# haoheliu/voicefixer_main

Measured on NVIDIA H100. Metric: clips_per_sec_10s_44k1, higher is better.
Workload: dtype f16 tensor-core (UNet: hi/lo split, fp32-grade; vocoder: hi-only), f32 accumulate

## Files before the change

voicefixer_main_b200/csrc/gemm_tc.cu:

```cuda
#include "gemm.cuh"
#include "ptx.cuh"

namespace vf {

namespace {

constexpr int kRowValid = 1, kRowPad = 2;

struct RowInfo {
  uint32_t orow;
  uint32_t flags;
};


__device__ __forceinline__ void epi_bar_sync(int nthreads) {
  asm volatile("bar.sync 1, %0;" ::"r"(nthreads) : "memory");
}
__device__ __forceinline__ void wg_bar_sync(int wg) {
  asm volatile("bar.sync %0, 128;" ::"r"(2 + wg) : "memory");
}

struct ChunkDesc {
  int a_c;
  int a_off;
  uint32_t kk;
  uint32_t flags;
};

struct TileCoord {
  int nt, mi, img;
  __device__ __forceinline__ TileCoord(uint32_t tile, const GemmTcParams& P, int n_tiles, int m_tiles) {
    const uint32_t mt = fast_div(tile, (uint32_t)n_tiles, P.magic_n);
    nt = (int)(tile - mt * (uint32_t)n_tiles);
    const uint32_t im = fast_div(mt, (uint32_t)m_tiles, P.magic_m);
    img = (int)im;
    mi = (int)(mt - im * (uint32_t)m_tiles);
  }
};

}

__device__ __forceinline__ void pack_hi(const float (&v)[32], uint32_t (&hi)[16]) {
#pragma unroll
  for (int i = 0; i < 16; ++i) {
    const __half2 h = __floats2half2_rn(v[2 * i], v[2 * i + 1]);
    hi[i] = *reinterpret_cast<const uint32_t*>(&h);
  }
}
__device__ __forceinline__ void pack_hi_lo(const float (&v)[32], uint32_t (&hi)[16], uint32_t (&lo)[16]) {
#pragma unroll
  for (int i = 0; i < 16; ++i) {
    const __half2 h = __floats2half2_rn(v[2 * i], v[2 * i + 1]);
    hi[i] = *reinterpret_cast<const uint32_t*>(&h);
    lo[i] = residual_h2(v[2 * i], v[2 * i + 1], hi[i]);
  }
}

template <bool TWO>
__device__ __forceinline__ void pack8(const float (&v)[32], const int i, uint4& h, uint4& l) {
  uint32_t hw[4], lw[4];
#pragma unroll
  for (int k = 0; k < 4; ++k) {
    const __half2 h2 = __floats2half2_rn(v[8 * i + 2 * k], v[8 * i + 2 * k + 1]);
    hw[k] = *reinterpret_cast<const uint32_t*>(&h2);
    if (TWO) lw[k] = residual_h2(v[8 * i + 2 * k], v[8 * i + 2 * k + 1], hw[k]);
  }
  h = make_uint4(hw[0], hw[1], hw[2], hw[3]);
  if (TWO) l = make_uint4(lw[0], lw[1], lw[2], lw[3]);
}

constexpr int GEMM_THREADS = 384;
constexpr int EPI_WARPS = 8;

template <int BN, int BK, bool THREE>
__global__ void __launch_bounds__(GEMM_THREADS, 1)
    gemm_tc_kernel(const __grid_constant__ GemmTcParams P) {
  constexpr int B_BYTES = BN * BK * 2;
  constexpr int ROW_BYTES = BK * 2;
  constexpr int EPI_THREADS = 32 * EPI_WARPS;
  constexpr int CHUNK_STEP = 2;
  constexpr int ACC_N = THREE ? 2 * BN : BN;
  constexpr uint32_t DHI = make_smem_desc_hi(ROW_BYTES);

  extern __shared__ __align__(16) uint8_t smem_raw[];
  uint8_t* smem = smem_raw + ((1024u - (smem_u32(smem_raw) & 1023u)) & 1023u);
  const int stages = P.stages;
  const int planes_a = P.planes_a;
  constexpr int B_SLOT = (THREE ? 2 : 1) * B_BYTES;
  constexpr int A_BOX_BYTES = GEMM_BM * ROW_BYTES;
  const int off_b = planes_a * A_BOX_BYTES;
  const int stage_bytes = off_b + B_SLOT;
  uint8_t* stg_base = smem + (size_t)stages * stage_bytes;
  uint8_t* rstg_base = stg_base + EPI_WARPS * 4096;
  uint8_t* tail = rstg_base + (size_t)P.resid_tma * EPI_WARPS * 4096;
  uint64_t* full_bar = reinterpret_cast<uint64_t*>(tail);
  uint64_t* empty_bar = full_bar + stages;
  uint64_t* resid_bar = empty_bar + stages;
  float* s_bias = reinterpret_cast<float*>(resid_bar + 16);
  float* s_scale = s_bias + BN;
  float* s_shift = s_scale + BN;
  float* s_head = s_shift + BN;
  RowInfo* s_rows = reinterpret_cast<RowInfo*>(s_head + 32);
  ChunkDesc* s_tab = reinterpret_cast<ChunkDesc*>(s_rows + EPI_WARPS * 32);

  const GemmProblem& pr = P.prob;
  const GemmEpilogue& e = pr.epi;
  const int warp = __shfl_sync(0xffffffffu, (int)(threadIdx.x >> 5), 0);
  const int lane = threadIdx.x & 31;
  const int n_tiles = pr.N / BN;
  const int total_tiles = pr.n_img * pr.m_tiles * n_tiles;
  const int tile_chunks = P.tile_chunks;
  const int seg_chunks = THREE ? P.seg_chunks : tile_chunks;

  if (warp == 0 && lane == 0) {
    for (int s = 0; s < stages; ++s) {
      mbar_init(full_bar + s, 1);
      mbar_init(empty_bar + s, EPI_WARPS);
    }
    for (int i = 0; i < 16; ++i) mbar_init(resid_bar + i, 1);
    fence_mbar_init();
    tma_prefetch_desc(&P.a_hi[0]);
    tma_prefetch_desc(&P.b_hi);
    if (!THREE) tma_prefetch_desc(&P.a_lo[0]);
  }
  for (int ci = threadIdx.x; ci < tile_chunks; ci += blockDim.x) {
    int t = 0, first = 0;
    for (; t < pr.ntaps - 1; ++t) {
      const int n = pr.taps[t].nch / BK * ((!THREE && pr.taps[t].both) ? 2 : 1);
      if (ci < first + n) break;
      first += n;
    }
    const GemmTap& tap = pr.taps[t];
    const int nk = tap.nch / BK;
    const bool lo_pass = !THREE && tap.both && ci - first >= nk;
    const int c = (ci - first - (lo_pass ? nk : 0)) * BK;
    ChunkDesc cd;
    cd.a_c = tap.c_off + c;
    cd.a_off = tap.a_off;
    cd.kk = (uint32_t)(tap.k_off + c);
    cd.flags = (uint32_t)(tap.src & 1) | (lo_pass ? 16u : 0u);
    s_tab[ci] = cd;
  }
  __syncthreads();

  if (warp < 4) {
    asm volatile("setmaxnreg.dec.sync.aligned.u32 40;\n" ::: "memory");
    if (warp == 0 && elect_one()) {
    int s = 0;
    uint32_t ph = 0;
    bool ok = true;
    for (int tile = blockIdx.x; tile < total_tiles && ok; tile += gridDim.x) {
      const TileCoord it((uint32_t)tile, P, n_tiles, pr.m_tiles);
      const int img = it.img;
      const int m0 = it.mi * GEMM_BM;
      const int n0 = it.nt * BN;
      const int nchunks = tile_is_empty(e, img, m0) ? 0 : tile_chunks;
      ChunkDesc cd = s_tab[0];
      for (int ci = 0; ci < nchunks; ++ci) {
        const ChunkDesc cur = cd;
        cd = s_tab[ci + 1 < tile_chunks ? ci + 1 : 0];
        if (!mbar_wait(empty_bar + s, ph ^ 1, e.err, ERR_PIPE_PRODUCER)) { ok = false; break; }
        const bool lo_pass = (cur.flags & 16u) != 0;
        const int src = cur.flags & 1u;
        uint8_t* st = smem + (size_t)s * stage_bytes;
        mbar_expect_tx(full_bar + s, (THREE ? 2u : 1u) * A_BOX_BYTES + B_SLOT);
        const int k0 = cur.kk;
        if (THREE) {
          tma_load_4d(st, &P.a_hi[src], full_bar + s, cur.a_c, m0 + cur.a_off, img, 0);
          tma_load_3d(st + off_b, &P.b_hi, full_bar + s, k0, n0, 0);
        } else {
          tma_load_3d(st, lo_pass ? &P.a_lo[src] : &P.a_hi[src], full_bar + s, cur.a_c, m0 + cur.a_off, img);
          tma_load_2d(st + off_b, &P.b_hi, full_bar + s, k0, n0);
        }
        if (++s == stages) { s = 0; ph ^= 1; }
      }
    }
    }
    __syncwarp();
  } else {
    asm volatile("setmaxnreg.inc.sync.aligned.u32 232;\n" ::: "memory");
    const int ew = warp - 4;
    const int wg = ew >> 2;
    const int wq = ew & 3;
    const int q = 2 * wg + (wq & 1);
    const int half = wq >> 1;
    float4* stg_f = reinterpret_cast<float4*>(stg_base) + (size_t)ew * 256;
    uint4* stg_h = reinterpret_cast<uint4*>(stg_f);
    uint4* stg_l = stg_h + 128;
    RowInfo* rows = s_rows + ew * 32;
    const int et = threadIdx.x - 128;
    float* stg_wg = reinterpret_cast<float*>(stg_base) + (size_t)wg * 4 * 1024;
    const int map = e.map, Wp = e.Wp, cout = e.cout, rows_in = e.rows_in;
    const bool has_affine = THREE && e.a_scale != nullptr, has_bias = e.bias != nullptr;
    const bool want_a = e.out_a.hi != nullptr, want_r = e.out_r.hi != nullptr, want_raw = THREE && e.out_raw != nullptr;
    const bool has_resid = THREE && e.resid != nullptr, has_resid_planes = e.resid_hi != nullptr, has_head = THREE && e.head_w != nullptr;
    const int act = e.act;
    const float slope = e.slope;
    const uint32_t resid_ar = THREE ? 0u : e.resid_ar, out_ar = THREE ? 0u : e.out_ar;
    const int h_row = lane >> 2, h_c16 = lane & 3;
    const int so_h0 = lane * 4, so_hx = (lane >> 1) & 3;
    const int sr_h0 = h_row * 4, sr_hx = h_c16;
    const int so_f0 = lane * 8, so_fx = lane & 7;
#define SO_H(i) (so_h0 + ((i) ^ so_hx))
#define SR_H(i) (32 * (i) + sr_h0 + (sr_hx ^ ((h_row >> 1) & 3)))
#define SO_F(i) (so_f0 + ((i) ^ so_fx))
    const bool convt1d_tma = map == MAP_CONVT1D && e.tma_out != 0;
    bool st_pending = false;
    auto stg_release = [&]() {
      if (st_pending) {
        if (lane == 0) tma_store_wait_read();
        __syncwarp();
        st_pending = false;
      }
    };
    const int resid_ring = P.resid_tma;
    uint8_t* rstg = rstg_base + (size_t)ew * resid_ring * 4096;
    uint64_t* rbar = resid_bar + ew * 2;
    uint32_t r_cons = 0, r_issued = 0;
    int pf_tile = blockIdx.x, pf_j = half;
    auto issue_resid = [&]() {
      if (pf_tile >= total_tiles) return;
      if (lane == 0) {
        const TileCoord pt((uint32_t)pf_tile, P, n_tiles, pr.m_tiles);
        const uint32_t slot = r_issued & (uint32_t)(resid_ring - 1);
        uint8_t* dst = rstg + slot * 4096;
        mbar_expect_tx(rbar + slot, 4096);
        if (THREE && e.resid != nullptr) tma_load_3d(dst, &P.i_res, rbar + slot, pt.nt * BN + pf_j * 32, pt.mi * GEMM_BM + q * 32, pt.img);
        else tma_load_4d(dst, &P.i_res, rbar + slot, pt.nt * BN + pf_j * 32, pt.mi * GEMM_BM + q * 32, pt.img, 0);
      }
      ++r_issued;
      pf_j += CHUNK_STEP;
      if (pf_j >= BN / 32) { pf_j = half; pf_tile += gridDim.x; }
    };
    if (half < BN / 32)
      for (int i = 0; i < resid_ring; ++i) issue_resid();
    int prev_n0 = -1, s = 0;
    uint32_t ph = 0;
    float amax = 0.f;
    bool ok = true;
    for (int tile = blockIdx.x; tile < total_tiles; tile += gridDim.x) {
      const TileCoord it((uint32_t)tile, P, n_tiles, pr.m_tiles);
      const int img = it.img;
      const int m0 = it.mi * GEMM_BM;
      const int n0 = it.nt * BN;
      if (n0 != prev_n0) {
        epi_bar_sync(EPI_THREADS);
        for (int i = et; i < BN; i += EPI_THREADS) {
          s_bias[i] = has_bias ? __ldg(e.bias + n0 + i) : 0.f;
          int co = n0 + i;
          if (map != MAP_PLAIN) co -= (co / cout) * cout;
          s_scale[i] = has_affine ? __ldg(e.a_scale + co) : 1.f;
          s_shift[i] = has_affine ? __ldg(e.a_shift + co) : 0.f;
        }
        if (et < 32) s_head[et] = has_head ? __ldg(e.head_w + et) : 0.f;
        epi_bar_sync(EPI_THREADS);
        prev_n0 = n0;
      }
      const int wrow0 = m0 + q * 32;
      const int r = wrow0 + lane;
      const bool row_ok = r < rows_in;
      float head_acc = 0.f;
      int cth = 0, ctw = 0;
      uint32_t orow = 0, flags = 0;
      if (map == MAP_PLAIN) {
        if (row_ok) flags = kRowValid | (((Wp > 0 && (r % Wp) == Wp - 1) || r >= valid_rows(e.row_valid, img)) ? kRowPad : 0);
      } else if (map == MAP_CONVT2D) {
        cth = r / Wp;
        ctw = r - cth * Wp;
      }
      auto store_rows_h = [&](const OutPlane& op, const int co0, const bool two, const CUtensorMap* tm) {
        if (map == MAP_PLAIN) {
          fence_proxy_async();
          __syncwarp();
          if (lane == 0) {
            tma_store_4d(tm, stg_h, op.c_off + co0, e.out_row0 + wrow0, img, 0);
            tma_store_commit();
          }
          st_pending = true;
        } else {
#pragma unroll
          for (int i = 0; i < 4; ++i) {
            const RowInfo ri = rows[8 * i + h_row];
            if (ri.flags & kRowValid) {
              const size_t o = (size_t)ri.orow * op.ld + op.c_off + co0;
              reinterpret_cast<uint4*>(op.hi + o)[h_c16] = stg_h[SR_H(i)];
              if (two) reinterpret_cast<uint4*>(op.lo + o)[h_c16] = stg_l[SR_H(i)];
            }
          }
        }
      };

      auto process_chunk = [&](const int j, float (&v)[32]) {
        const int nb = n0 + j * 32;
        int co0 = nb;
        if (map != MAP_PLAIN) {
          const int phase = nb / cout;
          co0 = nb - phase * cout;
          orow = 0; flags = 0;
          if (row_ok) {
            const int vrows = valid_rows(e.row_valid, img);
            if (map == MAP_CONVT2D) {
              const int ph = phase >> 1, pw = phase & 1;
              const int col = 2 * ctw + pw;
              if (col < e.ct_out_wp) {
                orow = (uint32_t)((size_t)img * e.out_img_rows + (size_t)(2 * cth + ph) * e.ct_out_wp + col);
                flags = kRowValid | ((col == e.ct_out_wp - 1 || r >= vrows) ? kRowPad : 0);
              } else if (r >= vrows) {
                flags = kRowPad;
              }
            } else {
              const long t = (long)r * e.ct_stride + phase - e.ct_pad;
              if (t >= 0 && t < e.out_rows_valid) {
                orow = (uint32_t)((size_t)img * e.out_img_rows + e.out_row0 + t);
                flags = kRowValid | (t >= vrows ? kRowPad : 0);
              }
            }
          }
          __syncwarp();
          rows[lane] = RowInfo{orow, flags};
        }
        if (has_bias) {
          const float4* bp = reinterpret_cast<const float4*>(s_bias + j * 32);
#pragma unroll
          for (int i = 0; i < 8; ++i) {
            const float4 b4 = bp[i];
            v[4 * i] += b4.x; v[4 * i + 1] += b4.y; v[4 * i + 2] += b4.z; v[4 * i + 3] += b4.w;
          }
        }
        if (THREE && has_resid) {
          const uint32_t slot = r_cons & (uint32_t)(resid_ring - 1);
          if (ok && !mbar_wait(rbar + slot, (r_cons >> (resid_ring >> 1)) & 1u, e.err, ERR_PIPE_EPILOGUE)) ok = false;
          ++r_cons;
          const float4* rt = reinterpret_cast<const float4*>(rstg + slot * 4096);
#pragma unroll
          for (int i = 0; i < 8; ++i) {
            const float4 x = rt[SO_F(i)];
            v[4 * i] += x.x; v[4 * i + 1] += x.y; v[4 * i + 2] += x.z; v[4 * i + 3] += x.w;
          }
          __syncwarp();
          issue_resid();
        }
        if (has_resid_planes) {
          const uint32_t slot = r_cons & (uint32_t)(resid_ring - 1);
          if (ok && !mbar_wait(rbar + slot, (r_cons >> (resid_ring >> 1)) & 1u, e.err, ERR_PIPE_EPILOGUE)) ok = false;
          ++r_cons;
          const uint4* rth = reinterpret_cast<const uint4*>(rstg + slot * 4096);
          const uint4* rtl = rth + 128;
#pragma unroll
          for (int i = 0; i < 4; ++i) {
            const uint4 xh = rth[SO_H(i)], xl = rtl[SO_H(i)];
            const __half2* ph = reinterpret_cast<const __half2*>(&xh);
            const __half2* pl = reinterpret_cast<const __half2*>(&xl);
#pragma unroll
            for (int k = 0; k < 4; ++k)
              add_planes(v[8 * i + 2 * k], v[8 * i + 2 * k + 1], reinterpret_cast<const uint32_t*>(ph)[k], reinterpret_cast<const uint32_t*>(pl)[k], resid_ar);
          }
          __syncwarp();
          issue_resid();
        }
        const bool pad = (flags & kRowPad) != 0;
        if (pad) {
#pragma unroll
          for (int i = 0; i < 32; ++i) v[i] = 0.f;
        }
        if (THREE && want_raw) {
          stg_release();
          __syncwarp();
#pragma unroll
          for (int i = 0; i < 8; ++i) stg_f[SO_F(i)] = make_float4(v[4 * i], v[4 * i + 1], v[4 * i + 2], v[4 * i + 3]);
          fence_proxy_async();
          __syncwarp();
          if (lane == 0) {
            tma_store_3d(&P.o_raw, stg_f, co0, e.out_row0 + wrow0, img);
            tma_store_commit();
          }
          st_pending = true;
        }
        if (want_r) {
          stg_release();
          __syncwarp();
#pragma unroll
          for (int i = 0; i < 4; ++i) {
            uint4 h, l;
            pack8<true>(v, i, h, l);
            stg_h[SO_H(i)] = h;
            stg_l[SO_H(i)] = l;
          }
          __syncwarp();
          store_rows_h(e.out_r, co0, true, &P.o_r);
        }
        if (has_head) {
#pragma unroll
          for (int i = 0; i < 32; ++i) head_acc = fmaf(v[i], s_head[i], head_acc);
        }
        if (want_a) {
          if (has_affine) {
            const float4* sc = reinterpret_cast<const float4*>(s_scale + j * 32);
            const float4* sh = reinterpret_cast<const float4*>(s_shift + j * 32);
#pragma unroll
            for (int i = 0; i < 8; ++i) {
              const float4 a4 = sc[i], b4 = sh[i];
              v[4 * i] = fmaf(v[4 * i], a4.x, b4.x); v[4 * i + 1] = fmaf(v[4 * i + 1], a4.y, b4.y);
              v[4 * i + 2] = fmaf(v[4 * i + 2], a4.z, b4.z); v[4 * i + 3] = fmaf(v[4 * i + 3], a4.w, b4.w);
            }
          }
          if (out_ar) {
            if (row_ok) {
#pragma unroll
              for (int i = 0; i < 32; ++i) amax = fmaxf(amax, fabsf(v[i]));
            }
            stg_release();
            __syncwarp();
#pragma unroll
            for (int i = 0; i < 4; ++i) {
              uint32_t h4[4], l4[4];
#pragma unroll
              for (int k = 0; k < 4; ++k) {
                const float v0 = pad ? 0.f : v[8 * i + 2 * k], v1 = pad ? 0.f : v[8 * i + 2 * k + 1];
                ar_split(v0, v1, fmaxf(v0, v0 * slope), fmaxf(v1, v1 * slope), out_ar, h4[k], l4[k]);
              }
              stg_h[SO_H(i)] = make_uint4(h4[0], h4[1], h4[2], h4[3]);
              stg_l[SO_H(i)] = make_uint4(l4[0], l4[1], l4[2], l4[3]);
            }
          } else {
            if (act == ACT_LRELU) {
#pragma unroll
              for (int i = 0; i < 32; ++i) v[i] = fmaxf(v[i], v[i] * slope);
            } else if (act == ACT_ELU) {
#pragma unroll
              for (int i = 0; i < 32; ++i) v[i] = v[i] > 0.f ? v[i] : expm1f(v[i]);
            }
            if (pad) {
#pragma unroll
              for (int i = 0; i < 32; ++i) v[i] = 0.f;
            }
            if (row_ok) {
#pragma unroll
              for (int i = 0; i < 32; ++i) amax = fmaxf(amax, fabsf(v[i]));
            }
            stg_release();
            __syncwarp();
#pragma unroll
            for (int i = 0; i < 4; ++i) {
              uint4 h, l;
              pack8<THREE>(v, i, h, l);
              stg_h[SO_H(i)] = h;
              if (THREE) stg_l[SO_H(i)] = l;
            }
          }
          __syncwarp();
          if (convt1d_tma && !(wrow0 == 0 && nb / cout < e.ct_pad)) {
            fence_proxy_async();
            __syncwarp();
            if (lane == 0) {
              const int d = nb / cout - e.ct_pad;
              const int up = d < 0 ? 1 : 0;
              tma_store_5d(&P.o_a, stg_h, e.out_a.c_off + co0, d + up * e.ct_stride, wrow0 - up, img, 0);
              tma_store_commit();
            }
            st_pending = true;
          } else {
            store_rows_h(e.out_a, co0, THREE || out_ar, &P.o_a);
          }
        }
      };

      float acc[ACC_N / 2];
      float acc2[THREE ? BN / 2 : 1];
      float tot[THREE ? BN / 2 : 1];
      {
        int left_in_seg = 0, prev_s = -1;
        uint32_t started = 0;
        bool first_seg = true;
        const int nchunks = tile_is_empty(e, img, m0) ? 0 : tile_chunks;
        for (int ci = 0; ci < nchunks; ++ci) {
          if (THREE && left_in_seg == 0) {
            left_in_seg = min(seg_chunks, tile_chunks - ci);
            started = 0;
          }
          if (ok && !mbar_wait(full_bar + s, ph, e.err, ERR_PIPE_EPILOGUE)) ok = false;
          const uint32_t da_hi = make_smem_desc_lo(smem_u32(smem + (size_t)s * stage_bytes + wg * 64 * ROW_BYTES));
          const uint32_t da_lo = da_hi + (uint32_t)(A_BOX_BYTES >> 4);
          const uint32_t db = make_smem_desc_lo(smem_u32(smem + (size_t)s * stage_bytes + off_b));
          wgmma_fence_regs(acc, ACC_N / 2);
          if (THREE) wgmma_fence_regs(acc2, BN / 2);
          wgmma_fence();
#pragma unroll
          for (int k = 0; k < BK / 16; ++k) {
            Wgmma<ACC_N>::mma(acc, smem_desc(da_hi + 2 * k, DHI), smem_desc(db + 2 * k, DHI), k == 0 ? started : 1u);
            if (THREE) Wgmma<BN>::mma(acc2, smem_desc(da_lo + 2 * k, DHI), smem_desc(db + 2 * k, DHI), k == 0 ? started : 1u);
          }
          wgmma_commit();
          started = 1;
          const bool close_seg = THREE ? (--left_in_seg == 0) : (ci + 1 == tile_chunks);
          if (close_seg) {
            wgmma_wait<0>();
            wgmma_fence_regs(acc, ACC_N / 2);
            if (THREE) wgmma_fence_regs(acc2, BN / 2);
            __syncwarp();
            if (lane == 0) {
              if (prev_s >= 0) mbar_arrive(empty_bar + prev_s);
              mbar_arrive(empty_bar + s);
            }
            prev_s = -1;
            if (THREE) {
#pragma unroll
              for (int i = 0; i < BN / 2; ++i) tot[i] = (first_seg ? 0.f : tot[i]) + (acc[i] + (acc[BN / 2 + i] + acc2[i]));
              first_seg = false;
            }
          } else {
            wgmma_wait<1>();
            wgmma_fence_regs(acc, ACC_N / 2);
            if (THREE) wgmma_fence_regs(acc2, BN / 2);
            __syncwarp();
            if (prev_s >= 0 && lane == 0) mbar_arrive(empty_bar + prev_s);
            prev_s = s;
          }
          if (++s == stages) { s = 0; ph ^= 1; }
        }
        wgmma_wait<0>();
        wgmma_fence_regs(acc, ACC_N / 2);
      }
      const float* fin = THREE ? tot : acc;
#pragma unroll
      for (int rd = 0; rd < (BN + 63) / 64; ++rd) {
        stg_release();
        wg_bar_sync(wg);
#pragma unroll
        for (int i = 0; i < BN / 2; i += 2) {
          const int col = 8 * (i / 4) + 2 * (lane & 3);
          if ((8 * (i / 4)) / 64 != rd) continue;
          const int row = 16 * wq + (lane >> 2) + 8 * ((i / 2) & 1);
          const int cc = (col >> 5) & 1, c32 = col & 31;
          const int rr = row & 31;
          float* tile_p = stg_wg + (size_t)(2 * cc + (row >> 5)) * 1024;
          *reinterpret_cast<float2*>(tile_p + rr * 32 + ((((c32 >> 2) ^ (rr & 7)) << 2) | (c32 & 3))) = make_float2(fin[i], fin[i + 1]);
        }
        wg_bar_sync(wg);
        const int j = 2 * rd + half;
        if (j < BN / 32) {
          float v[32];
#pragma unroll
          for (int i = 0; i < 8; ++i) {
            const float4 x = stg_f[SO_F(i)];
            v[4 * i] = x.x; v[4 * i + 1] = x.y; v[4 * i + 2] = x.z; v[4 * i + 3] = x.w;
          }
          __syncwarp();
          process_chunk(j, v);
        }
      }
      if (THREE && half == 0) epilogue_head(e, img, r, head_acc);
    }
    if ((map == MAP_PLAIN || convt1d_tma) && lane == 0) tma_store_wait_all();
    if (!(amax <= 65504.f) && e.err) atomicCAS(e.err, 0, ERR_FP16_OVERFLOW);
  }
}

size_t gemm_tc_smem_bytes(int bn, int bk, int stages, int planes_a, int terms, int tile_chunks, int resid_tma) {
  const size_t stage = (size_t)planes_a * GEMM_BM * bk * 2 + (size_t)(terms == 3 ? 2 : 1) * bn * bk * 2;
  return stages * stage + EPI_WARPS * 4096 * (1 + resid_tma) + (2 * stages + 16) * 8 + (3 * bn + 32) * 4 + EPI_WARPS * 32 * 8 +
         (size_t)tile_chunks * 16 + 1024;
}

template <int BN, int BK, bool THREE>
static cudaError_t launch_cfg(const GemmTcParams& p, cudaStream_t stream) {
  const size_t smem = gemm_tc_smem_bytes(BN, BK, p.stages, p.planes_a, p.prob.terms, p.tile_chunks, p.resid_tma);
  static bool attr_set = false;
  if (!attr_set) {
    cudaError_t e = cudaFuncSetAttribute(gemm_tc_kernel<BN, BK, THREE>, cudaFuncAttributeMaxDynamicSharedMemorySize, 227 * 1024);
    if (e != cudaSuccess) return e;
    attr_set = true;
  }
  gemm_tc_kernel<BN, BK, THREE><<<p.grid, GEMM_THREADS, smem, stream>>>(p);
  return cudaGetLastError();
}
template <int BK>
static cudaError_t launch_bk(const GemmTcParams& p, int bn, cudaStream_t stream) {
  const bool three = p.prob.terms == 3;
  if (bn == 128) return three ? cudaErrorInvalidValue : launch_cfg<128, BK, false>(p, stream);
  if (bn == 64) return three ? launch_cfg<64, BK, true>(p, stream) : launch_cfg<64, BK, false>(p, stream);
  if (bn == 32) return three ? launch_cfg<32, BK, true>(p, stream) : launch_cfg<32, BK, false>(p, stream);
  return cudaErrorInvalidValue;
}

uint32_t gemm_tc_magic(uint32_t d, uint64_t nmax) {
  if (d <= 1) return 0u;
  if (nmax * (uint64_t)d >= (1ull << 32)) return 0xffffffffu;
  return (uint32_t)(((1ull << 32) + d - 1) / d);
}

int gemm_tc_max_bn(int terms) { return terms == 3 ? 64 : 128; }

cudaError_t launch_gemm_tc(const GemmTcParams& p, int bn, int bk, cudaStream_t stream) {
  if (bk == 64) return launch_bk<64>(p, bn, stream);
  if (bk == 32) return launch_bk<32>(p, bn, stream);
  return cudaErrorInvalidValue;
}

}
```

Measured before the change: 141.5.

## Add ping-pong warpgroup schedule for non-three-term GEMM tiles

For GEMMs that are not three-term and use no TMA residual, the two consumer warpgroups now take alternating tiles, each computing the full 128-row tile. Ordering barriers pass the MMA turn between them so one group's epilogue overlaps the other's tensor-core mainloop, replacing the cooperative split of each tile. This costs more registers (two accumulator halves per warpgroup), an extra output staging buffer and per-group bias arrays in shared memory, and adds barrier-ordering complexity.

After: 141.3, median of 6. About the same (-0.1%).

```diff
diff --git a/voicefixer_main_b200/csrc/gemm_tc.cu b/voicefixer_main_b200/csrc/gemm_tc.cu
--- a/voicefixer_main_b200/csrc/gemm_tc.cu
+++ b/voicefixer_main_b200/csrc/gemm_tc.cu
@@ -18,6 +18,12 @@
 }
 __device__ __forceinline__ void wg_bar_sync(int wg) {
   asm volatile("bar.sync %0, 128;" ::"r"(2 + wg) : "memory");
+}
+__device__ __forceinline__ void mma_turn_wait(int wg) {
+  asm volatile("bar.sync %0, 256;" ::"r"(4 + wg) : "memory");
+}
+__device__ __forceinline__ void mma_turn_pass(int wg) {
+  asm volatile("bar.arrive %0, 256;" ::"r"(5 - wg) : "memory");
 }
 
 struct ChunkDesc {
@@ -72,13 +78,16 @@
 constexpr int GEMM_THREADS = 384;
 constexpr int EPI_WARPS = 8;
 
-template <int BN, int BK, bool THREE>
+template <int BN, int BK, bool THREE, bool PP>
 __global__ void __launch_bounds__(GEMM_THREADS, 1)
     gemm_tc_kernel(const __grid_constant__ GemmTcParams P) {
+  static_assert(!(THREE && PP), "the 3-term kernels keep the cooperative schedule");
   constexpr int B_BYTES = BN * BK * 2;
   constexpr int ROW_BYTES = BK * 2;
-  constexpr int EPI_THREADS = 32 * EPI_WARPS;
-  constexpr int CHUNK_STEP = 2;
+  constexpr int EPI_THREADS = PP ? 128 : 32 * EPI_WARPS;
+  constexpr int CHUNK_STEP = PP ? 1 : 2;
+  constexpr int ROUND_COLS = 32 * CHUNK_STEP;
+  constexpr int HALVES = PP ? 2 : 1;
   constexpr int ACC_N = THREE ? 2 * BN : BN;
   constexpr uint32_t DHI = make_smem_desc_hi(ROW_BYTES);
 
@@ -92,12 +101,13 @@
   const int stage_bytes = off_b + B_SLOT;
   uint8_t* stg_base = smem + (size_t)stages * stage_bytes;
   uint8_t* rstg_base = stg_base + EPI_WARPS * 4096;
-  uint8_t* tail = rstg_base + (size_t)P.resid_tma * EPI_WARPS * 4096;
+  uint8_t* ostg_base = rstg_base + (size_t)P.resid_tma * EPI_WARPS * 4096;
+  uint8_t* tail = ostg_base + (PP ? EPI_WARPS * 4096 : 0);
   uint64_t* full_bar = reinterpret_cast<uint64_t*>(tail);
   uint64_t* empty_bar = full_bar + stages;
   uint64_t* resid_bar = empty_bar + stages;
   float* s_bias = reinterpret_cast<float*>(resid_bar + 16);
-  float* s_scale = s_bias + BN;
+  float* s_scale = s_bias + HALVES * BN;
   float* s_shift = s_scale + BN;
   float* s_head = s_shift + BN;
   RowInfo* s_rows = reinterpret_cast<RowInfo*>(s_head + 32);
@@ -115,7 +125,7 @@
   if (warp == 0 && lane == 0) {
     for (int s = 0; s < stages; ++s) {
       mbar_init(full_bar + s, 1);
-      mbar_init(empty_bar + s, EPI_WARPS);
+      mbar_init(empty_bar + s, PP ? 4 : EPI_WARPS);
     }
     for (int i = 0; i < 16; ++i) mbar_init(resid_bar + i, 1);
     fence_mbar_init();
@@ -182,13 +192,20 @@
     const int ew = warp - 4;
     const int wg = ew >> 2;
     const int wq = ew & 3;
-    const int q = 2 * wg + (wq & 1);
-    const int half = wq >> 1;
+    const int q = PP ? wq : 2 * wg + (wq & 1);
+    const int half = PP ? 0 : wq >> 1;
+    const int tile_stride = (PP ? 2 : 1) * gridDim.x;
     float4* stg_f = reinterpret_cast<float4*>(stg_base) + (size_t)ew * 256;
-    uint4* stg_h = reinterpret_cast<uint4*>(stg_f);
+    uint4* stg_h = PP ? reinterpret_cast<uint4*>(ostg_base) + (size_t)ew * 256
+                      : reinterpret_cast<uint4*>(stg_f);
     uint4* stg_l = stg_h + 128;
     RowInfo* rows = s_rows + ew * 32;
-    const int et = threadIdx.x - 128;
+    const int et = PP ? (threadIdx.x & 127) : threadIdx.x - 128;
+    float* const s_bias_g = s_bias + (PP ? wg * BN : 0);
+    auto epi_sync = [&]() {
+      if (PP) wg_bar_sync(wg);
+      else epi_bar_sync(EPI_THREADS);
+    };
     float* stg_wg = reinterpret_cast<float*>(stg_base) + (size_t)wg * 4 * 1024;
     const int map = e.map, Wp = e.Wp, cout = e.cout, rows_in = e.rows_in;
     const bool has_affine = THREE && e.a_scale != nullptr, has_bias = e.bias != nullptr;
@@ -217,7 +234,7 @@
     uint8_t* rstg = rstg_base + (size_t)ew * resid_ring * 4096;
     uint64_t* rbar = resid_bar + ew * 2;
     uint32_t r_cons = 0, r_issued = 0;
-    int pf_tile = blockIdx.x, pf_j = half;
+    int pf_tile = blockIdx.x + (PP ? wg * gridDim.x : 0), pf_j = half;
     auto issue_resid = [&]() {
       if (pf_tile >= total_tiles) return;
       if (lane == 0) {
@@ -230,7 +247,7 @@
       }
       ++r_issued;
       pf_j += CHUNK_STEP;
-      if (pf_j >= BN / 32) { pf_j = half; pf_tile += gridDim.x; }
+      if (pf_j >= BN / 32) { pf_j = half; pf_tile += tile_stride; }
     };
     if (half < BN / 32)
       for (int i = 0; i < resid_ring; ++i) issue_resid();
@@ -238,22 +255,30 @@
     uint32_t ph = 0;
     float amax = 0.f;
     bool ok = true;
-    for (int tile = blockIdx.x; tile < total_tiles; tile += gridDim.x) {
+    for (int tile = blockIdx.x, jt = 0; tile < total_tiles; tile += gridDim.x, ++jt) {
       const TileCoord it((uint32_t)tile, P, n_tiles, pr.m_tiles);
       const int img = it.img;
       const int m0 = it.mi * GEMM_BM;
       const int n0 = it.nt * BN;
+      const int nchunks = tile_is_empty(e, img, m0) ? 0 : tile_chunks;
+      if (PP && (jt & 1) != wg) {
+        s += nchunks;
+        while (s >= stages) { s -= stages; ph ^= 1; }
+        continue;
+      }
       if (n0 != prev_n0) {
-        epi_bar_sync(EPI_THREADS);
+        epi_sync();
         for (int i = et; i < BN; i += EPI_THREADS) {
-          s_bias[i] = has_bias ? __ldg(e.bias + n0 + i) : 0.f;
-          int co = n0 + i;
-          if (map != MAP_PLAIN) co -= (co / cout) * cout;
-          s_scale[i] = has_affine ? __ldg(e.a_scale + co) : 1.f;
-          s_shift[i] = has_affine ? __ldg(e.a_shift + co) : 0.f;
-        }
-        if (et < 32) s_head[et] = has_head ? __ldg(e.head_w + et) : 0.f;
-        epi_bar_sync(EPI_THREADS);
+          s_bias_g[i] = has_bias ? __ldg(e.bias + n0 + i) : 0.f;
+          if (THREE) {
+            int co = n0 + i;
+            if (map != MAP_PLAIN) co -= (co / cout) * cout;
+            s_scale[i] = has_affine ? __ldg(e.a_scale + co) : 1.f;
+            s_shift[i] = has_affine ? __ldg(e.a_shift + co) : 0.f;
+          }
+        }
+        if (THREE && et < 32) s_head[et] = has_head ? __ldg(e.head_w + et) : 0.f;
+        epi_sync();
         prev_n0 = n0;
       }
       const int wrow0 = m0 + q * 32;
@@ -320,7 +345,7 @@
           rows[lane] = RowInfo{orow, flags};
         }
         if (has_bias) {
-          const float4* bp = reinterpret_cast<const float4*>(s_bias + j * 32);
+          const float4* bp = reinterpret_cast<const float4*>(s_bias_g + j * 32);
 #pragma unroll
           for (int i = 0; i < 8; ++i) {
             const float4 b4 = bp[i];
@@ -465,38 +490,50 @@
         }
       };
 
-      float acc[ACC_N / 2];
+      float acc[HALVES][ACC_N / 2];
       float acc2[THREE ? BN / 2 : 1];
       float tot[THREE ? BN / 2 : 1];
+      auto fence_acc = [&]() {
+#pragma unroll
+        for (int h = 0; h < HALVES; ++h) wgmma_fence_regs(acc[h], ACC_N / 2);
+        if (THREE) wgmma_fence_regs(acc2, BN / 2);
+      };
       {
         int left_in_seg = 0, prev_s = -1;
         uint32_t started = 0;
         bool first_seg = true;
-        const int nchunks = tile_is_empty(e, img, m0) ? 0 : tile_chunks;
+        bool pass_turn = PP && tile + (int)gridDim.x < total_tiles;
+        if (PP && jt > 0) mma_turn_wait(wg);
+        const int a_row0 = PP ? 0 : wg * 64;
         for (int ci = 0; ci < nchunks; ++ci) {
           if (THREE && left_in_seg == 0) {
             left_in_seg = min(seg_chunks, tile_chunks - ci);
             started = 0;
           }
           if (ok && !mbar_wait(full_bar + s, ph, e.err, ERR_PIPE_EPILOGUE)) ok = false;
-          const uint32_t da_hi = make_smem_desc_lo(smem_u32(smem + (size_t)s * stage_bytes + wg * 64 * ROW_BYTES));
+          const uint32_t da_hi = make_smem_desc_lo(smem_u32(smem + (size_t)s * stage_bytes + a_row0 * ROW_BYTES));
           const uint32_t da_lo = da_hi + (uint32_t)(A_BOX_BYTES >> 4);
           const uint32_t db = make_smem_desc_lo(smem_u32(smem + (size_t)s * stage_bytes + off_b));
-          wgmma_fence_regs(acc, ACC_N / 2);
-          if (THREE) wgmma_fence_regs(acc2, BN / 2);
+          fence_acc();
           wgmma_fence();
 #pragma unroll
           for (int k = 0; k < BK / 16; ++k) {
-            Wgmma<ACC_N>::mma(acc, smem_desc(da_hi + 2 * k, DHI), smem_desc(db + 2 * k, DHI), k == 0 ? started : 1u);
+#pragma unroll
+            for (int h = 0; h < HALVES; ++h)
+              Wgmma<ACC_N>::mma(acc[h], smem_desc(da_hi + h * (64 * ROW_BYTES >> 4) + 2 * k, DHI), smem_desc(db + 2 * k, DHI),
+                                k == 0 ? started : 1u);
             if (THREE) Wgmma<BN>::mma(acc2, smem_desc(da_lo + 2 * k, DHI), smem_desc(db + 2 * k, DHI), k == 0 ? started : 1u);
           }
           wgmma_commit();
           started = 1;
+          if (pass_turn && ci + 1 == nchunks) {
+            mma_turn_pass(wg);
+            pass_turn = false;
+          }
           const bool close_seg = THREE ? (--left_in_seg == 0) : (ci + 1 == tile_chunks);
           if (close_seg) {
             wgmma_wait<0>();
-            wgmma_fence_regs(acc, ACC_N / 2);
-            if (THREE) wgmma_fence_regs(acc2, BN / 2);
+            fence_acc();
             __syncwarp();
             if (lane == 0) {
               if (prev_s >= 0) mbar_arrive(empty_bar + prev_s);
@@ -505,39 +542,43 @@
             prev_s = -1;
             if (THREE) {
 #pragma unroll
-              for (int i = 0; i < BN / 2; ++i) tot[i] = (first_seg ? 0.f : tot[i]) + (acc[i] + (acc[BN / 2 + i] + acc2[i]));
+              for (int i = 0; i < BN / 2; ++i) tot[i] = (first_seg ? 0.f : tot[i]) + (acc[0][i] + (acc[0][BN / 2 + i] + acc2[i]));
               first_seg = false;
             }
           } else {
             wgmma_wait<1>();
-            wgmma_fence_regs(acc, ACC_N / 2);
-            if (THREE) wgmma_fence_regs(acc2, BN / 2);
+            fence_acc();
             __syncwarp();
             if (prev_s >= 0 && lane == 0) mbar_arrive(empty_bar + prev_s);
             prev_s = s;
           }
           if (++s == stages) { s = 0; ph ^= 1; }
         }
+        if (pass_turn) mma_turn_pass(wg);
         wgmma_wait<0>();
-        wgmma_fence_regs(acc, ACC_N / 2);
-      }
-      const float* fin = THREE ? tot : acc;
-#pragma unroll
-      for (int rd = 0; rd < (BN + 63) / 64; ++rd) {
-        stg_release();
+        fence_acc();
+      }
+#pragma unroll
+      for (int rd = 0; rd < (BN + ROUND_COLS - 1) / ROUND_COLS; ++rd) {
+        if (!PP) stg_release();
         wg_bar_sync(wg);
 #pragma unroll
-        for (int i = 0; i < BN / 2; i += 2) {
-          const int col = 8 * (i / 4) + 2 * (lane & 3);
-          if ((8 * (i / 4)) / 64 != rd) continue;
-          const int row = 16 * wq + (lane >> 2) + 8 * ((i / 2) & 1);
-          const int cc = (col >> 5) & 1, c32 = col & 31;
-          const int rr = row & 31;
-          float* tile_p = stg_wg + (size_t)(2 * cc + (row >> 5)) * 1024;
-          *reinterpret_cast<float2*>(tile_p + rr * 32 + ((((c32 >> 2) ^ (rr & 7)) << 2) | (c32 & 3))) = make_float2(fin[i], fin[i + 1]);
+        for (int h = 0; h < HALVES; ++h) {
+          const float* fin = THREE ? tot : acc[h];
+#pragma unroll
+          for (int i = 0; i < BN / 2; i += 2) {
+            const int col = 8 * (i / 4) + 2 * (lane & 3);
+            if ((8 * (i / 4)) / ROUND_COLS != rd) continue;
+            const int row = 64 * h + 16 * wq + (lane >> 2) + 8 * ((i / 2) & 1);
+            const int c32 = col & 31;
+            const int rr = row & 31;
+            const int t = PP ? (row >> 5) : 2 * ((col >> 5) & 1) + (row >> 5);
+            float* tile_p = stg_wg + (size_t)t * 1024;
+            *reinterpret_cast<float2*>(tile_p + rr * 32 + ((((c32 >> 2) ^ (rr & 7)) << 2) | (c32 & 3))) = make_float2(fin[i], fin[i + 1]);
+          }
         }
         wg_bar_sync(wg);
-        const int j = 2 * rd + half;
+        const int j = CHUNK_STEP * rd + half;
         if (j < BN / 32) {
           float v[32];
 #pragma unroll
@@ -556,30 +597,38 @@
   }
 }
 
+static bool gemm_tc_pingpong(int terms, int resid_tma) { return terms != 3 && resid_tma == 0; }
+
 size_t gemm_tc_smem_bytes(int bn, int bk, int stages, int planes_a, int terms, int tile_chunks, int resid_tma) {
   const size_t stage = (size_t)planes_a * GEMM_BM * bk * 2 + (size_t)(terms == 3 ? 2 : 1) * bn * bk * 2;
-  return stages * stage + EPI_WARPS * 4096 * (1 + resid_tma) + (2 * stages + 16) * 8 + (3 * bn + 32) * 4 + EPI_WARPS * 32 * 8 +
-         (size_t)tile_chunks * 16 + 1024;
-}
-
-template <int BN, int BK, bool THREE>
+  const int pp = gemm_tc_pingpong(terms, resid_tma) ? 1 : 0;
+  return stages * stage + EPI_WARPS * 4096 * (1 + pp + resid_tma) + (2 * stages + 16) * 8 + ((1 + pp + 2) * bn + 32) * 4 +
+         EPI_WARPS * 32 * 8 + (size_t)tile_chunks * 16 + 1024;
+}
+
+template <int BN, int BK, bool THREE, bool PP>
 static cudaError_t launch_cfg(const GemmTcParams& p, cudaStream_t stream) {
   const size_t smem = gemm_tc_smem_bytes(BN, BK, p.stages, p.planes_a, p.prob.terms, p.tile_chunks, p.resid_tma);
   static bool attr_set = false;
   if (!attr_set) {
-    cudaError_t e = cudaFuncSetAttribute(gemm_tc_kernel<BN, BK, THREE>, cudaFuncAttributeMaxDynamicSharedMemorySize, 227 * 1024);
+    cudaError_t e = cudaFuncSetAttribute(gemm_tc_kernel<BN, BK, THREE, PP>, cudaFuncAttributeMaxDynamicSharedMemorySize, 227 * 1024);
     if (e != cudaSuccess) return e;
     attr_set = true;
   }
-  gemm_tc_kernel<BN, BK, THREE><<<p.grid, GEMM_THREADS, smem, stream>>>(p);
+  gemm_tc_kernel<BN, BK, THREE, PP><<<p.grid, GEMM_THREADS, smem, stream>>>(p);
   return cudaGetLastError();
+}
+template <int BN, int BK>
+static cudaError_t launch_hi(const GemmTcParams& p, cudaStream_t stream) {
+  return gemm_tc_pingpong(p.prob.terms, p.resid_tma) ? launch_cfg<BN, BK, false, true>(p, stream)
+                                                     : launch_cfg<BN, BK, false, false>(p, stream);
 }
 template <int BK>
 static cudaError_t launch_bk(const GemmTcParams& p, int bn, cudaStream_t stream) {
   const bool three = p.prob.terms == 3;
-  if (bn == 128) return three ? cudaErrorInvalidValue : launch_cfg<128, BK, false>(p, stream);
-  if (bn == 64) return three ? launch_cfg<64, BK, true>(p, stream) : launch_cfg<64, BK, false>(p, stream);
-  if (bn == 32) return three ? launch_cfg<32, BK, true>(p, stream) : launch_cfg<32, BK, false>(p, stream);
+  if (bn == 128) return three ? cudaErrorInvalidValue : launch_hi<128, BK>(p, stream);
+  if (bn == 64) return three ? launch_cfg<64, BK, true, false>(p, stream) : launch_hi<64, BK>(p, stream);
+  if (bn == 32) return three ? launch_cfg<32, BK, true, false>(p, stream) : launch_hi<32, BK>(p, stream);
   return cudaErrorInvalidValue;
 }
 
```
